# EI-CoreBioinformatics/portcullis

Measured on AMD Instinct MI355X. Metric: junc_reads_per_sec, higher is better.
Workload: dtype int32; 1 GPU; BASELINE configs[2]: synthetic 199999998 paired-end 150-bp reads, 25 contigs of GRCh38 lengths (3088286401 bp), 249999 junctions, orientation FR; reads_total=199999998, junctions_total=249999, contigs=25, reads_rank0=199999998, pairs_rank0=66692850

## Files before the change

### portcullis_amd/csrc/pjb_api.hip

```cpp
#include "pjb_host.hip.h"
#include "pjb_kernels.hip.h"
#include "pjb_chain.hip.h"

static int slot_init(pjb_ctx *c, int k);
static void aux_streams(pjb_ctx *c) {
    if (!c->stream3) (void)hipStreamCreateWithFlags(&c->stream3, hipStreamNonBlocking);
    if (!c->stream4) (void)hipStreamCreateWithFlags(&c->stream4, hipStreamNonBlocking);
}

extern "C" {

namespace {
std::mutex g_host_mu;
std::map<void *, size_t> g_host_registered;
}
void *pjb_host_alloc(size_t bytes) {
    if (bytes >= ((size_t)8 << 20)) {
        const size_t huge = (size_t)2 << 20, len = (bytes + huge - 1) & ~(huge - 1);
        void *p = mmap(nullptr, len, PROT_READ | PROT_WRITE, MAP_PRIVATE | MAP_ANONYMOUS, -1, 0);
        if (p != MAP_FAILED) {
            (void)madvise(p, len, MADV_HUGEPAGE);
            const size_t nt = std::min<size_t>(4, len >> 24);
            auto touch = [&](size_t t) {
                const size_t per = ((len / std::max<size_t>(nt, 1)) + huge - 1) & ~(huge - 1), a = std::min(len, per * t), b = std::min(len, a + per);
// ... 99 lines not shown
        (void)hipFuncSetAttribute((const void *)rs_scatter<0, u64>, hipFuncAttributeMaxDynamicSharedMemorySize, (int)rs_scatter_lds_bytes(RS_MAX_BITS));
        (void)hipFuncSetAttribute((const void *)rs_scatter<0, u32>, hipFuncAttributeMaxDynamicSharedMemorySize, (int)rs_scatter_lds_bytes(RS_MAX_BITS, 4));
    };
    std::thread attr_thread(attributes);
    struct JoinAttr {
        std::thread &t;
        ~JoinAttr() {
            if (t.joinable()) t.join();
        }
    } join_attr{attr_thread};
    c->cfg = *cfg;
    memset(&c->timing, 0, sizeof c->timing);
    e = hipStreamCreateWithFlags(&c->stream, hipStreamNonBlocking);
    if (e != hipSuccess) {
        delete c;
        return fail(nullptr, PJB_ERR_HIP, "hipStreamCreate: %s", hipGetErrorString(e));
    }
    if (!(cfg->flags & PJB_FLAG_NO_CHAINS)) aux_streams(c);
    (void)hipEventCreateWithFlags(&c->ev_front, hipEventDisableTiming);
    c->scan_tiles = &c->b_scan_tiles;
    cmark("main streams");
    if (!(cfg->flags & PJB_FLAG_NO_CHAINS))
        for (int k = 0; k < 4 && k < PJB_MAX_QUEUED; k++) (void)slot_init(c, k);
    cmark("chain slots");
    c->inflate_lanes = std::max(1, n_cu) * (160 * 1024 / ingest_lds_bytes()) * 64;
    c->ktime = (cfg->flags & PJB_FLAG_KERNEL_TIMING) != 0;
    c->extra = (cfg->flags & PJB_FLAG_EXTRA) != 0;
    if (const char *s = getenv("PJB_K1_SERIAL")) c->k1_serial = atoi(s) != 0;
    if (const char *s = getenv("PJB_K1S_BLOCKS")) c->k1s_blocks_forced = std::max(0, std::min(atoi(s), (int)K1S_BLOCKS));
    if (const char *s = getenv("PJB_RADIX_BITS")) {
        int v = atoi(s);
        if (v >= 4 && v <= RS_MAX_BITS) c->radix_max_bits = v;
    }
    cmark("options");
    attr_thread.join();
    cmark("kernel attributes");
    *out = c;
    return PJB_OK;
}


void pjb_destroy(pjb_ctx *c) {
    if (!c) return;
    (void)hipSetDevice(c->cfg.device);
    (void)hipDeviceSynchronize();
    (void)exhume(c);
#ifdef K1E_PROF
    {
        unsigned long long h[16] = {0};
        (void)hipDeviceSynchronize();
        if (hipMemcpyFromSymbol(h, HIP_SYMBOL(pjb::g_k1e_prof), sizeof h) == hipSuccess) {
            unsigned long long tot = 0;
            for (int i = 0; i < 12; i++) tot += h[i];
            static const char *nm[12] = {"block start", "prologue", "shapes (wait ops)", "windows issue", "next records issue", "stage wait", "next ops issue", "compare+emit", "lists", "cand flush", "span of bases", "bases issue"};
            for (int i = 0; i < 12; i++) fprintf(stderr, "[k1e_prof] %-20s %6.2f %%  %llu\n", nm[i], tot ? 100.0 * (double)h[i] / (double)tot : 0.0, h[i]);
        }
    }
#endif
    while (!c->open.empty()) close_contig(c, c->open.begin()->first);
    extra_clear(c);
    for (auto &kv : c->filter_keys)
        if (kv.second.first) (void)hipFree(kv.second.first);
    c->filter_keys.clear();
    for (auto &g : c->contigs) free_contig(g);
    for (auto &b : c->genome_pool) release(b);
    c->genome_pool.clear();
    for (auto &sl : c->slab_pool)
        if (sl.p) (void)hipFree(sl.p);
    if (c->rows_pinned) (void)hipHostFree(c->rows_pinned);
    if (c->rows_table) (void)hipFree(c->rows_table);
    bam_stage_clear(c);
    for (int k = 0; k < PJB_MAX_QUEUED; k++) {
        CtlSlot &S = c->sl[k];
        if (S.pub) (void)hipHostFree(S.pub);
        if (S.batches_pinned) (void)hipHostFree(S.batches_pinned);
        for (auto &ev : S.ev)
            if (ev) (void)hipEventDestroy(ev);
        if (S.ev_rows) (void)hipEventDestroy(S.ev_rows);
        if (S.ev_done) (void)hipEventDestroy(S.ev_done);
        Buf *sb[] = {&S.x_q, &S.x_spos, &S.x_send, &S.x_gapoff, &S.x_zlist, &S.x_scnt, &S.x_codes, &S.cstats, &S.err, &S.gencount, &S.batches, &S.rows, &S.tile_cnt, &S.tile_stats, &S.splidx, &S.splpoff, &S.splrec, &S.tile_soff, &S.chunk_tile, &S.scan_parts, &S.members, &S.okey, &S.g,
                     &S.rec, &S.jidbam, &S.jkey, &S.total, &S.bitmap, &S.wrank, &S.pagecnt, &S.pagerank, &S.ends, &S.firstid,
                     &S.key[0], &S.key[1], &S.idx[0], &S.idx[1], &S.hist, &S.hist_scan, &S.hist_part, &S.bintotal, &S.scan_tiles, &S.jid, &S.seg, &S.runfirst,
                     &S.runstart, &S.ent, &S.entsum, &S.frag, &S.fragj, &S.masks, &S.acc, &S.ancl, &S.ancr, &S.genlist, &S.runs};
        for (Buf *b : sb) release(*b);
        hipEvent_t evs[] = {S.ev_k1, S.ev_xk1, S.ev_fork, S.ev_join, S.ev_fork2, S.ev_join2};
        for (hipEvent_t e : evs)
            if (e) (void)hipEventDestroy(e);
        if (S.main) (void)hipStreamDestroy(S.main);
// ... 911 lines not shown
        if (b > a) c->ktime_only.push_back(s.substr(a, b - a));
        a = b + 1;
    }
    return PJB_OK;
}

int pjb_reset_kernel_timing(pjb_ctx *c) {
    if (!c) return PJB_ERR_ARG;
    std::fill(c->kcount.begin(), c->kcount.end(), 0);
    std::fill(c->kms.begin(), c->kms.end(), 0.0);
    return PJB_OK;
}

int pjb_set_option(pjb_ctx *c, const char *name, int64_t value) {
    if (!c || !name) return PJB_ERR_ARG;
    if (c->n_fl) return fail(c, PJB_ERR_STATE, "set_option: target %d is still queued", c->fl[0].tid);
    const std::string n = name;
    if (n == "overlap") c->side_stream = value != 0;
    else if (n == "dense_ids") c->dense_ids = value != 0;
    else if (n == "extra_dense") c->extra_dense_only = value != 0;
    else if (n == "sort_floor") c->sort_floor = (u32)std::max<int64_t>(1, std::min<int64_t>(value, 1 << 30));
    else if (n == "window_skip") c->window_skip = value != 0;
    else if (n == "run_sort") c->run_sort = value != 0;
    else if (n == "run_window") {
        if (value < 0 || value > (int64_t)RUN_W) return fail(c, PJB_ERR_ARG, "set_option: run_window takes 0 (the default, %u) to %u", RUN_W, RUN_W);
        c->run_window = (u32)value;
    } else if (n == "grow_batch") {
        if (value < 0 || value > 32768) return fail(c, PJB_ERR_ARG, "set_option: grow_batch takes 0 (the default: what the pool holds) to 32768 trees");
        c->model.grow_batch = (u32)value;
    } else if (n == "knn_chunk") {
        if (value < 0 || value > (1 << 22)) return fail(c, PJB_ERR_ARG, "set_option: knn_chunk takes 0 (the default: sized to fill the chip) to %d base rows", 1 << 22);
        c->model.knn_chunk = (u32)value;
    } else if (n == "list_cap") c->list_cap_forced = (u32)std::max<int64_t>(0, std::min<int64_t>(value, 1 << 30));
    else return fail(c, PJB_ERR_ARG, "set_option: unknown option '%s'", name);
    return PJB_OK;
}

int pjb_get_timing(const pjb_ctx *c, pjb_timing *out) {
    if (!c || !out) return PJB_ERR_ARG;
    if (c->cfg.abi_version >= 4) *out = c->timing;
    else memcpy(out, &c->timing, offsetof(pjb_timing, repeats));
    return PJB_OK;
}

}
```

### portcullis_amd/csrc/pjb_chain.hip.h

```cpp
#pragma once

constexpr unsigned K6_BLOCKS = 128;

static size_t rows_upper_bound(const pjb_ctx *c) {
    size_t n = c->rows_n;
    for (int k = 0; k < c->n_fl; k++)
        if (c->fl[k].queued) n += c->fl[k].lim.junc_limit;
    return n;
}

static void wait_flight(pjb_ctx *c, Flight &f) {
    if (f.queued) (void)hipEventSynchronize(c->sl[f.slot].ev_done);
}

static int rows_table_reserve(pjb_ctx *c, Flight &f, u32 JL) {
    size_t old = rows_upper_bound(c);
    if (old + JL <= c->rows_cap) return PJB_OK;
    for (int k = 0; k < c->n_fl; k++)
        if (c->fl[k].queued && &c->fl[k] != &f) wait_flight(c, c->fl[k]);
    int rc = rows_sync(c);
    if (rc) return rc;
    old = std::min(old, c->rows_cap);
    const size_t ncap = std::max<size_t>((old + JL) * 3 / 2, 1024);
    pjb_junction_row *nd = nullptr;
// ... 338 lines not shown
    }
    LAUNCH(c, "k1_scan_tiles", k1_scan_tiles, dim3(c->k1s_blocks_forced ? (u32)c->k1s_blocks_forced : k1s_blocks(n_tiles)), dim3(K1S_THREADS), (u32 *)S.tile_cnt.p, (const TileStats *)S.tile_stats.p,
           n_tiles, ch.d_cs, ch.PL, kf, ch.group ? INT32_MAX - 1 : ch.ref_len, (const u64 *)nullptr, (u32 *)S.tile_soff.p, (u32 *)S.chunk_tile.p,
           (ScanPart *)S.scan_parts.p, ++S.scan_epoch, c->window_skip ? 1u : 0u);
    EmitLists el;
    el.cand = f.lim.dense ? (u64 *)S.key[1].p : (u64 *)nullptr;
    el.bitmap = f.lim.dense ? (u64 *)S.bitmap.p : (u64 *)nullptr;
    el.page_cnt = f.lim.dense ? (u32 *)S.pagecnt.p : (u32 *)nullptr;
    el.cand_anc = (u64 *)S.ent.p;
    el.gen_list = (u64 *)S.genlist.p;
    el.gen_cnt = ch.d_gen_cnt;
    el.gen_cap = ch.gen_cap;
    el.pack_nn = ch.pack_nn;
    for (size_t b0 = 0; b0 < batches.size(); b0 += K1E_MAXB) {
        const size_t nb = std::min<size_t>(K1E_MAXB, batches.size() - b0);
        u64 reads = 0;
        for (size_t bi = b0; bi < b0 + nb; bi++) reads += (u64)batches[bi].n;
        const u32 nt = (u32)std::min<u64>((reads + K1_TILE - 1) / K1_TILE + nb, 0x7fffffffu);
        static const u32 tiles_per_block = getenv("PJB_K1E_TILES") ? (u32)std::max(1, atoi(getenv("PJB_K1E_TILES"))) : 8u;
        const u32 grid = std::max<u32>(1, std::min<u32>(nt, std::max<u32>(1024, nt / tiles_per_block)));
        LAUNCH(c, "k1_emit", k1_emit, dim3(grid), dim3(256), (const DevBatch *)S.batches.p + b0, (int)nb, n_tiles, (const u32 *)S.tile_cnt.p,
               (const u32 *)S.tile_soff.p, (const u32 *)S.chunk_tile.p, (const u32 *)S.splidx.p, (const u32 *)S.splpoff.p, (const uint4 *)S.splrec.p, ch.pr, el, kf,
               GT, ch.fast_codes ? 1 : 0, (int)c->cfg.orientation, ch.d_err, ch.d_cs);
    }
    if (c->k1_serial && !k1_late) {
        HIP_TRY(c, hipEventRecord(S.ev_k1, st));
        c->last_k1_ev = S.ev_k1;
    }
    if (ch.group)
        LAUNCH(c, "kg_member_stats", kg_member_stats, dim3((unsigned)ch.n_members), dim3(256), (const u32 *)S.tile_cnt.p, (const TileStats *)S.tile_stats.p,
               (const u32 *)ch.d_tile_lo, ch.n_members, ch.d_members, n_tiles, (const ContigStats *)ch.d_cs);
    LAUNCH(c, "k1_generic", k1_generic, dim3(std::min<u32>(std::max<u32>(1, (u32)(((u64)ch.gen_cap * GEN_SHARDS + K1E_T - 1) / K1E_T)), 1536u )), dim3(K1E_T),
           (const DevBatch *)S.batches.p, (int)batches.size(), (const u32 *)S.splidx.p, (const uint4 *)S.splrec.p, ch.pr, el, kf, GT, ch.fast_codes ? 1 : 0,
           (int)c->cfg.orientation, ch.d_err, ch.d_cs);
    if (c->k1_serial && k1_late) {
        HIP_TRY(c, hipEventRecord(S.ev_k1, st));
        c->last_k1_ev = S.ev_k1;
    }
    STAGE_EVENT(1);
    return PJB_OK;
}

static int chain_k4b(Chain &ch) {
    pjb_ctx *c = ch.c;
    CtlSlot &S = ch.S;
    const u32 gen_grid = std::min<u32>(2 * (u32)(((u64)ch.gen_cap * GEN_SHARDS + 255) / 256), 2560u);
    LAUNCH(c, "k4b_generic", k4b_generic, dim3(gen_grid), dim3(256), (const u64 *)S.genlist.p, (const u32 *)ch.d_gen_cnt, ch.gen_cap, (const u64 *)ch.pr.key,
           ch.pr.rec, (const u32 *)S.jidbam.p, ch.kf, (const DevBatch *)S.batches.p, (int)ch.f.batches.size(), (const int32_t *)S.ancl.p, (const int32_t *)S.ancr.p,
           ch.GT, ch.any_x ? 1 : 0, ch.any_x ? 0 : 1, ch.d_err, (const ContigStats *)ch.d_cs, ch.pack_nn, (const u32 *)S.splidx.p, (const uint4 *)S.splrec.p);
    return PJB_OK;
}

static int chain_k2d(Chain &ch) {
    pjb_ctx *c = ch.c;
    Flight &f = ch.f;
    CtlSlot &S = ch.S;
    if (!f.lim.dense) return PJB_OK;
    const KeyFmt kf = ch.kf;
    const u32 JL = ch.JL;
    const size_t n_words = ch.n_words;
    int rc;
    const u32 cand_blocks = std::min<u32>(ch.pair_blocks, 1024u);
    const u64 *okey = (const u64 *)ch.pr.key;
    u64 *cand = (u64 *)S.key[1].p;
    const u32 n_pages = (u32)((n_words + ((size_t)1 << KD_PAGE_SHIFT) - 1) >> KD_PAGE_SHIFT);
    if ((rc = run_scan(c, "kd_rank", ArrU32Fn{(const u32 *)S.pagecnt.p}, ExclusiveU32Sink{(u32 *)S.pagerank.p}, (u64)n_pages, (u64 *)S.total.p)))
        return rc;
// ... 241 lines not shown
```

### portcullis_amd/csrc/pjb_device.hip.h

```cpp
#pragma once

#include <hip/hip_runtime.h>
#include <stdint.h>

#include "../../include/portcullis_amd.h"

namespace pjb {

typedef unsigned long long u64;
typedef unsigned int u32;

struct DevBatch {
    const int32_t *pos;
    const uint16_t *flag;
    const uint8_t *mapq;
    const uint8_t *xs;
    const int32_t *l_qseq;
    const int32_t *mtid;
    const int32_t *mpos;
    const uint32_t *cig_off;
    const uint32_t *cigar;
    const uint32_t *seq_off;
    const uint8_t *seq4;
    const u64 *name_hash;
// ... 64 lines not shown
__device__ __forceinline__ void rec_store(PairRec *dst, const PairRec &r) {
    uint4 *q = reinterpret_cast<uint4 *>(dst);
    q[0] = make_uint4((u32)r.aux, (u32)(r.aux >> 32), (u32)r.lstart, (u32)r.rend);
    q[1] = make_uint4((u32)r.pos, (u32)r.aend, r.meta, r.updown);
}
__device__ __forceinline__ PairRec rec_load(const PairRec *src) {
    const uint4 *q = reinterpret_cast<const uint4 *>(src);
    const uint4 a = q[0], b = q[1];
    PairRec r;
    r.aux = (u64)a.x | ((u64)a.y << 32);
    r.lstart = (int32_t)a.z;
    r.rend = (int32_t)a.w;
    r.pos = (int32_t)b.x;
    r.aend = (int32_t)b.y;
    r.meta = b.z;
    r.updown = b.w;
    return r;
}

enum : u32 {
    META_CAT_MASK = 3u,
    META_MULTI = 1u << 2,
    META_XS_SHIFT = 3,
    META_UM = 1u << 5,
    META_BPP = 1u << 6,
    META_PPP = 1u << 7,
    META_REL = 1u << 8,
    META_SIMPLE = 1u << 9,
};
__device__ __forceinline__ u64 pack_res(u32 minMatch, u32 mmes, u32 mis) {
    return (u64)(minMatch & 0xfffffu) | ((u64)(mmes & 0xfffffu) << 20) | ((u64)mis << 40);
}
constexpr u32 RES_FIELD_MAX = 0xfffffu;

constexpr int GROUP_MAX = 32;
constexpr int32_t GROUP_GAP = 4096;
struct GroupTab {
    int32_t n;
    int32_t voff[GROUP_MAX];
    int32_t len[GROUP_MAX];
    int32_t tid[GROUP_MAX];
    const uint8_t *d[GROUP_MAX];
    const u32 *codes[GROUP_MAX];
    const u32 *codes2[GROUP_MAX];
    u32 exc_members;
};
struct Member {
    int32_t idx, voff, len, tid;
    const uint8_t *d;
    const u32 *codes;
};
__device__ __forceinline__ Member member_of(const GroupTab &T, int32_t vpos) {
    int m = 0;
    if (T.n > 1) {
#pragma unroll
        for (int s = GROUP_MAX / 2; s >= 1; s >>= 1)
            if (m + s < T.n && T.voff[m + s] <= vpos) m += s;
    }
    Member M;
    M.idx = m;
    M.voff = T.voff[m];
    M.len = T.len[m];
    M.tid = T.tid[m];
    M.d = T.d[m];
    M.codes = T.codes[m];
    return M;
// ... 427 lines not shown
```

### portcullis_amd/csrc/pjb_host.hip.h

```cpp
#pragma once
#include "pjb_device.hip.h"
#include "pjb_extra_types.hip.h"

#include <algorithm>
#include <sys/mman.h>
#include <thread>
#include <chrono>
#include <cstdarg>
#include <cstdio>
#include <cstdlib>
#include <cstring>
#include <map>
#include <memory>
#include <mutex>
#include <string>
#include <thread>
#include <vector>

using namespace pjb;


inline thread_local std::string g_create_error;
inline thread_local std::string g_thread_error;
inline thread_local const void *g_thread_error_ctx = nullptr;
// ... 224 lines not shown
    std::vector<Slab> slab_pool;
    uint8_t *stage[2] = {nullptr, nullptr};
    size_t stage_cap[2] = {0, 0};
    hipEvent_t stage_ev[2] = {nullptr, nullptr};
    bool stage_busy[2] = {false, false};
    unsigned stage_next = 0;
    pjb_junction_row *rows_pinned = nullptr;
    pjb_junction_row *rows_table = nullptr;
    bool rows_copy_pending = false;
    int last_slot = 0;
    int inflate_lanes = 512 * 64;
    bool side_stream = true;
    bool dense_ids = true;
    u32 junc_seen = 0;
    int lbits_seen = 18;
    size_t rows_n = 0, rows_cap = 0;
    size_t rows_pinned_cap = 0;
    std::vector<void *> graveyard;
    std::mutex grave_mu;
    size_t last_rows_n = 0;
    uint8_t *mirror = nullptr;
    size_t mirror_cap = 0;
    int64_t *mirror_hdr = nullptr;
    size_t mirror_rows = 0;
    int64_t mirror_acc[5] = {0, 0, 0, INT32_MAX, 0};
    pjb_timing timing;
    int radix_max_bits = 11;
    double junc_per_read = 0;
    u32 sort_floor = 1u << 16;
    bool window_skip = true;
    bool run_sort = true;
    u32 run_window = 0;
    u32 list_cap_forced = 0;
    bool k1_serial = true;
    hipEvent_t last_k1_ev = nullptr;
    int k1s_blocks_forced = 0;
    bool ktime = false;
    std::vector<std::string> knames;
    std::vector<int64_t> kcount;
    std::vector<double> kms;
    std::vector<std::string> ktime_only;
    Buf *scan_tiles = nullptr;
    Buf b_scan_tiles;
    Buf b_inf_comp, b_inf_out, b_inf_blocks, b_inf_status, b_inf_scratch, b_inf_bitmap;
    Buf b_dfl_in, b_dfl_sym, b_dfl_slots, b_dfl_size, b_dfl_off, b_dfl_packed;
    Buf b_bam_seg, b_bam_rec, b_bam_ctl;
    struct IndexState *index = nullptr;
    bool extra = false;
    std::vector<ExtraContig> xc;
    std::map<int32_t, std::pair<u64 *, u32>> filter_keys;
    Buf f_pos, f_cigoff, f_cigar, f_codes;
    ModelState model;
    Buf x_pos, x_endx, x_q, x_prefq, x_ce, x_bound, x_de, x_dropped, x_zlist, x_cnt, x_tabk, x_tabc, x_rs, x_re, x_rr, x_tileoff;
    Buf x_xrall, x_tab;
    size_t x_tab_slots = 0, x_tab_n = 0;
    XArena xarena;
    pjb_extra_row *xrows_pinned = nullptr;
    size_t xrows_pinned_cap = 0;
    bool extra_dense_only = false;
    Buf b_hasx, b_xtotal;
    Buf b_fasta_raw;
};


inline int fail(pjb_ctx *c, int code, const char *fmt, ...) {
    char tmp[1024];
// ... 316 lines not shown
```

### portcullis_amd/csrc/pjb_kernels.hip.h

```cpp
#pragma once

#include "pjb_device.hip.h"

namespace pjb {

__global__ __launch_bounds__(256) void k0_upper(uint8_t *g, int64_t n, int do_upper, int *has_x) {
    int64_t i = ((int64_t)blockIdx.x * 256 + threadIdx.x) * 16;
    bool x = false;
    for (int64_t j = i; j < n && j < i + 16; j++) {
        uint8_t c = g[j];
        x |= (c == 'X' || (do_upper && c == 'x'));
    }
    if (__ballot(x) && lane_id() == 0) atomicOr(has_x, 1);
    if (!do_upper) return;
    if (i + 16 <= n && ((uintptr_t)(g + i) & 15) == 0) {
        uint4 v = *reinterpret_cast<uint4 *>(g + i);
        u32 *w = reinterpret_cast<u32 *>(&v);
#pragma unroll
        for (int k = 0; k < 4; k++) {
            u32 x = w[k], r = 0;
#pragma unroll
            for (int b = 0; b < 4; b++) {
                u32 c = (x >> (8 * b)) & 0xff;
                if (c >= 'a' && c <= 'z') c -= 32;
// ... 878 lines not shown
}
constexpr int GEN_MAXB = 256;
struct BatchTab {
    u32 tbase[GEN_MAXB], seqw[GEN_MAXB], cigw[GEN_MAXB];
    __device__ __forceinline__ void fill(const DevBatch *batches, int n_batches) {
        if ((int)threadIdx.x < n_batches && threadIdx.x < (u32)GEN_MAXB) {
            const PJB_GLOBAL DevBatch *d = as_global(batches + threadIdx.x);
            tbase[threadIdx.x] = d->tile_base;
            seqw[threadIdx.x] = as_global(d->seq_off)[d->n];
            cigw[threadIdx.x] = as_global(d->cig_off)[d->n];
        }
    }
    __device__ __forceinline__ int find(const DevBatch *batches, int n_batches, u32 tile) const {
        int lo = 0, hi = n_batches - 1;
        if (n_batches <= GEN_MAXB) {
            while (lo < hi) {
                const int mid = (lo + hi + 1) >> 1;
                if (tbase[mid] <= tile) lo = mid;
                else hi = mid - 1;
            }
        } else {
            while (lo < hi) {
                const int mid = (lo + hi + 1) >> 1;
                if (gload(&batches[mid].tile_base) <= tile) lo = mid;
                else hi = mid - 1;
            }
        }
        return lo;
    }
    __device__ __forceinline__ u32 seq_words(const DevBatch &b, int bi) const { return bi < GEN_MAXB ? seqw[bi] : gload(b.seq_off + b.n); }
    __device__ __forceinline__ u32 cig_words(const DevBatch &b, int bi) const { return bi < GEN_MAXB ? cigw[bi] : gload(b.cig_off + b.n); }
};

struct NCursor {
    u32 i;
    int32_t acc;
    bool has;
    int32_t peek;
};
template <typename Ops>
__device__ __forceinline__ void ncursor_advance(NCursor &c, const Ops cig, u32 n) {
    c.has = false;
    while (c.i < n) {
        u32 op = cig[c.i++];
        u32 ty = op & 15u;
        if (op_consumes_ref(ty)) c.acc += (int32_t)(op >> 4);
        if (ty == OP_N) {
            c.has = true;
            c.peek = c.acc;
            return;
        }
    }
}

constexpr int SIMPLE_NW = 8;
struct CmpBlock {
    int32_t len, mism, first, last;
};
__device__ __forceinline__ u64 cmp_blocks_res(const CmpBlock &L, const CmpBlock &R) {
    const u32 upM = L.last < 0 ? (u32)L.len : (u32)(L.len - 1 - L.last);
    const u32 downM = R.first < 0 ? (u32)R.len : (u32)R.first;
    const u32 tu = (u32)(L.len - L.mism), td = (u32)(R.len - R.mism);
    return pack_res(upM < downM ? upM : downM, tu < td ? tu : td, (u32)(L.mism + R.mism));
}
struct EmitRead {
    u32 n;
// ... 58 lines not shown
            if (rStart - 1 >= ref_len) rStart = ref_len - 1;
            const int32_t iend = rStart - 1;
            while (U.has && U.peek < istart) {
                cntU++;
                ncursor_advance(U, cig, n);
            }
            while (D.has && D.peek <= iend + 1) {
                cntD++;
                ncursor_advance(D, cig, n);
            }
            const int64_t idx = (int64_t)R.off + k;
            const u64 key = make_key(kf, istart, iend);
            P.key[idx] = key;
            if (P.g) P.g[idx] = g;
            pend.lstart = lStart;
            pend.updown = cntU | ((nN - cntD) << 16);
            if (lStart > istart) set_error(err, g, PJB_ERR_MIN_ANCHOR);
            prev = idx;
            prev_key = key;
            blkL = blk;
            blk = Block{0, 0, -1, -1};
            prevIstart = istart;
            prevQ = qAcc;
            prevIend = iend;
            prevRStartU = rStartU;
            sumAfter = 0;
            lStart = rStart;
            lEndExc = rStart;
            k++;
        } else {
            if (closed && ty != OP_S) {
                const bool cq = op_consumes_query(ty), cr = op_consumes_ref(ty);
                if (cq && cr)
                    cmp_words<SIMPLE_NW, true>(R.closed_seqw, qAcc, R.q_limit, R.gcodes, lEndExc - R.voff, (R.glen + 7) / 8 + 1, ln, blk.len, blk.mism, blk.first, blk.last);
                else {
                    blk.mism += ln;
                    if (blk.first < 0) blk.first = blk.len;
                    blk.last = blk.len + ln - 1;
                }
                blk.len += ln;
            }
            if (op_consumes_ref(ty)) {
                lEndExc += ln;
                sumAfter += ln;
            }
        }
        if (op_consumes_query(ty)) qAcc += ln;
    }
    if (prev >= 0) {
        int32_t rEndExc = prevRStartU + sumAfter;
        if (rEndExc - 1 >= ref_len) rEndExc = ref_len;
        pend.rend = rEndExc - 1;
        if (closed) pend.aux = closed_stats();
        rec_store(P.rec + prev, pend);
        on_pair(prev_key, pend.lstart, pend.rend);
        if (rEndExc - 1 < prevIend) set_error(err, g, PJB_ERR_MIN_ANCHOR);
    }
}

__device__ __forceinline__ u32 read_meta(u32 flag, u32 xs, u32 mapq, int32_t pos, int32_t mtid, int32_t mpos, int32_t tid, int orientation) {
    const bool pp_check = orientation == PJB_OR_FR || orientation == PJB_OR_RF || orientation == PJB_OR_FF;
    const bool first = flag & 0x40, rev = flag & 0x10;
    u32 meta = (first ? 0u : 2u) + (rev ? 1u : 0u);
    meta |= (xs & 3u) << META_XS_SHIFT;
    const bool um = mapq >= 30;
    if (um) meta |= META_UM;
    if (flag & 0x2) meta |= META_BPP;
    bool ppp = false;
    if (pp_check) {
        const bool paired = flag & 0x1, mate_mapped = !(flag & 0x8);
        if (paired && mate_mapped && tid == mtid) {
            const bool mrev = flag & 0x20;
            const bool diff = rev != mrev;
            const bool gap = !rev ? pos < mpos : pos > mpos;
            ppp = orientation == PJB_OR_FR ? (diff && gap) : orientation == PJB_OR_RF ? (diff && !gap) : (!diff && gap);
        }
    }
    if (ppp) meta |= META_PPP;
    if (um && (!pp_check || ppp)) meta |= META_REL;
    return meta;
}

constexpr int K1E_LOOK = 16;
#ifndef K1E_WAVES
#define K1E_WAVES 4
#endif
constexpr int K1E_T = 256, K1E_SHIFT = 8;
constexpr int KC_SLOTS = K1E_T;
constexpr u64 KD_EMPTY = ~0ull;
// ... 348 lines not shown
            const u32 n = O.n;
            const u32 (&op)[OPS_LDS] = O.op;
            g = b.base + R.r;
            off = R.toff + R.poff;
            meta = read_meta(O.flag, O.xs, O.mapq, pos, O.mtid, O.mpos, tid, orientation);
            const bool seq_ok = (R.sr.w & 0x8000u) != 0;
            if (gcodes != nullptr && n >= 3 && n <= 7) {
                const bool clipF = (op[0] & 15u) == OP_S;
                const u32 i0 = clipF ? 1u : 0u;
                const u32 oa = clipF ? op[1] : op[0], on_ = clipF ? op[2] : op[1], ob = clipF ? op[3] : op[2];
                const u32 o3 = clipF ? op[4] : op[3], o4 = clipF ? op[5] : op[4], o5 = clipF ? op[6] : op[5];
                two = n >= i0 + 5u && (o3 & 15u) == OP_N;
                const u32 body = i0 + (two ? 5u : 3u);
                const u32 oL = two ? o5 : o3;
                const bool clipL = n == body + 1u && (oL & 15u) == OP_S;
                if (n == body || clipL) {
                    dS = clipF ? op[0] >> 4 : 0u;
                    const u32 dE = clipL ? oL >> 4 : 0u;
                    a = oa >> 4;
                    nl = on_ >> 4;
                    b2 = ob >> 4;
                    nl2 = two ? o3 >> 4 : 0u;
                    b3 = two ? o4 >> 4 : 0u;
                    simple = (oa & 15u) == OP_M && (on_ & 15u) == OP_N && (ob & 15u) == OP_M && a > 0 && b2 > 0 && a <= RES_FIELD_MAX && b2 <= RES_FIELD_MAX &&
                             dS <= RES_FIELD_MAX && lq > 1 && (u64)lq == (u64)dS + a + b2 + b3 + dE && seq_ok;
                    if (two)
                        simple = simple && (o4 & 15u) == OP_M && b3 > 0 && b3 <= RES_FIELD_MAX && nl > 0 && nl2 > 0 && pos >= 0 &&
                                 (int64_t)pos + a + nl + b2 + nl2 + b3 <= (int64_t)ref_len;
                }
            }
            two = two && simple;
            chk2 = two && window_reach(b2, nl, nl2, max_span);
            generic = !simple;
        }
        const u32 shard = (chunk >> (8 - K1E_SHIFT)) % GEN_SHARDS;
        const u32 base2 = ctx.list_reserve(2, chk2, 2u, shard), base3 = ctx.list_reserve(3, generic, 0u, shard);
        K1E_MARK(2);
        bool use2 = simple && gcodes2 != nullptr && !((O.excw >> (R.r & 31u)) & 1u) && pos >= 0 && (int64_t)pos + a + nl + b2 + nl2 + b3 <= (int64_t)ref_len &&
                    a <= (u32)C2_MAX_BLOCK && b2 <= (u32)C2_MAX_BLOCK && b3 <= (u32)C2_MAX_BLOCK;
        const int64_t n2w = codes2_words(ref_len);
        const bool any_exc = (G.exc_members >> mem) & 1u;
        Words2 x0 = {0, 0}, x1 = {0, 0}, x2 = {0, 0};
        if (use2 && any_exc) {
            const PJB_GLOBAL u32 *gexc = gcodes2 + n2w + K0_CODES2_PAD;
            const u32 g1 = (u32)pos + a + nl;
            x0 = gload_as<Words2>(gexc + ((u32)pos >> 11));
            x1 = gload_as<Words2>(gexc + (g1 >> 11));
            if (two) x2 = gload_as<Words2>(gexc + ((g1 + b2 + nl2) >> 11));
        }
        const bool more = v + 1 < v_hi, more2 = v + 2 < v_hi;
        EmitTrip T2 = T1;
        EmitRec R2 = R1;
        EmitOps On = O;
        if (more2) {
            T2 = locate(v + 2);
            R2 = fetch_rec(T2);
        }
        K1E_MARK(4);
        if (more) On = fetch_ops(T1, R1);
        K1E_MARK(6);
        const u32 *seqw = (const u32 *)b.seq4 + so;
        const int32_t q_limit = (int32_t)min(seq_words - 1u - so, 0x7fffffffu);
        if (simple) {
            const int32_t vpos = pos + voff;
            const int32_t aend_all = vpos + (int32_t)(a + nl + b2 + nl2 + b3) - 1;
            const u32 npairs = two ? 2u : 1u;
// ... 108 lines not shown
            for (u32 pr = 0; pr < 2; pr++) {
                if (pr >= npairs) break;
                PairRec Q;
                Q.lstart = lst_[pr];
                Q.rend = rend_[pr];
                Q.pos = vpos;
                Q.aend = aend_all;
                Q.meta = meta | META_SIMPLE | (two ? META_MULTI : 0u);
                Q.updown = ud_[pr];
                Q.aux = cmp_blocks_res(res[pr], res[pr + 1]);
                const u64 key = make_key(kf, ist_[pr], iend_[pr]);
                P.key[off + pr] = key;
                if (want_g) P.g[off + pr] = g;
                rec_store(P.rec + off + pr, Q);
                if (want_cand) cand_insert(key, Q.lstart, Q.rend);
            }
        }
        const u64 p1_entry = (u64)(E.pack_nn ? R.slot | (2u << 28) : R.slot) | ((u64)off << 32);
        K1E_MARK(7);
        ctx.list_write(2, chk2, base2, p1_entry, shard);
        ctx.list_write(3, generic, base3, (u64)R.slot | ((u64)off << 32), shard);
        K1E_MARK(8);
        if (!more) ctx.cand_flush(true);
        K1E_MARK(9);
        T = T1;
        R = R1;
        O = On;
        T1 = T2;
        R1 = R2;
    }
}

__global__ __launch_bounds__(K1E_T) void k1_generic(const DevBatch *batches, int n_batches, const u32 *spl_idx, const uint4 *spl_rec, Pairs P, EmitLists E, KeyFmt kf,
                                                    GroupTab G, int use_codes, int orientation, u64 *err, ContigStats *cs) {
    __shared__ EmitShared sh;
    __shared__ u32 s_ops[OPS_LDS][K1E_T];
    __shared__ u32 s_first[GEN_SHARDS + 1];
    __shared__ u32 s_wsum[4];
    __shared__ BatchTab s_bt;
    if (cs->P == 0) return;
    const u32 max_span = cs->max_span;
    const bool want_cand = E.cand != nullptr;
    EmitCtx ctx{sh, E, kf, cs, want_cand};
    ctx.init();
    static_assert(GEN_SHARDS == K1E_T, "a sub-list per thread");
    {
        const u32 c = E.gen_cnt[threadIdx.x * GEN_CNT_STRIDE + 4];
        s_bt.fill(batches, n_batches);
        u32 total;
        const u32 ex = block_escan<K1E_T / 64>(c < E.gen_cap ? c : E.gen_cap, s_wsum, &total);
        s_first[threadIdx.x] = ex;
        if (threadIdx.x == K1E_T - 1) s_first[GEN_SHARDS] = total;
        __syncthreads();
    }
    const u32 n_items = s_first[GEN_SHARDS];
    for (u32 item0 = blockIdx.x * K1E_T; item0 < n_items; item0 += gridDim.x * K1E_T) {
        const u32 item = item0 + threadIdx.x;
        u32 gen_pairs = 0, gen_kind = 0;
        u64 gen_entry = 0;
        if (item < n_items) {
            u32 sub = 0;
#pragma unroll
            for (u32 step = GEN_SHARDS / 2; step > 0; step >>= 1)
                if (sub + step < GEN_SHARDS && s_first[sub + step] <= item) sub += step;
            const u64 e3 = E.gen_list[((size_t)2 * GEN_SHARDS + sub) * E.gen_cap + (item - s_first[sub])];
            const u32 slot = (u32)e3;
            const int bi = s_bt.find(batches, n_batches, slot / (u32)K1_TILE);
            const DevBatch &b = batches[bi];
            const u32 r = spl_idx[slot];
            const uint4 sr = spl_rec[slot];
            const int m = b.member;
            const int32_t voff = G.voff[m], ref_len = G.len[m], vlen = voff + ref_len;
            const u32 *gcodes = use_codes ? G.codes[m] : (const u32 *)nullptr;
            EmitRead R;
            R.n = sr.w & 0x7fffu;
            if (R.n == 0x7fffu) R.n = gload(b.cig_off + r + 1) - sr.x;
            R.lq = (int32_t)(sr.w >> 16);
            if (R.lq == 0xffff) R.lq = gload(b.l_qseq + r);
            const int32_t pos = (int32_t)sr.y;
            R.pos = pos + voff;
            R.g = b.base + r;
            R.meta = read_meta(gload(b.flag + r), (u32)gload(b.xs + r), gload(b.mapq + r), pos, gload(b.mtid + r), gload(b.mpos + r), G.tid[m], orientation);
            R.seq_ok = (sr.w & 0x8000u) != 0;
            R.off = (u32)(e3 >> 32);
            OpsViewT<K1E_T, OPS_LDS> cig;
            cig.g = b.cigar + sr.x;
            cig.lds = &s_ops[0][threadIdx.x];
            {
                u32 w[OPS_LDS];
                fetch_ops8(as_global(b.cigar), sr.x, s_bt.cig_words(b, bi), w);
#pragma unroll
                for (int q = 0; q < OPS_LDS; q++) s_ops[q][threadIdx.x] = (u32)q < R.n ? w[q] : 0u;
            }
            u32 nN = 0, shape = 0;
            int32_t aligned = 0;
            int64_t qsum = 0, bsum = 0;
            u32 bref = 0, nl_prev = 0;
            bool reach = max_span == 0xffffffffu;
            for (u32 q = 0; q < R.n; q++) {
                const u32 o = cig[q], ty = o & 15u, ln = o >> 4;
                if (ty == OP_N) {
                    if (nN > 0) reach = reach || window_reach(bref, nl_prev, ln, max_span);
                    nl_prev = ln;
                    bref = 0;
                } else if (op_consumes_ref(ty))
                    bref = __builtin_elementwise_add_sat(bref, ln);
                nN += (ty == OP_N);
                if (op_consumes_ref(ty)) aligned += (int32_t)ln;
                if (op_consumes_query(ty)) qsum += ln;
                const bool len_ok = ln > 0 && ln <= RES_FIELD_MAX;
                if (ty == OP_M || ty == OP_EQ || ty == OP_X) shape = (shape == 0 || shape == 5 || shape == 2 || shape == 1 || shape == 6) && len_ok ? 1u : 4u;
                else if (ty == OP_I || ty == OP_D) shape = shape == 1 && len_ok ? 6u : 4u;
                else if (ty == OP_N) shape = shape == 1 && ln > 0 ? 2u : 4u;
                else if (ty == OP_S) shape = shape == 0 && len_ok ? 5u : shape == 1 && q + 1 == R.n ? 3u : 4u;
                else shape = 4;
                bsum = ty == OP_N ? 0 : ty == OP_S ? bsum : bsum + ln;
                if (bsum > (int64_t)RES_FIELD_MAX) shape = 4;
            }
            if (nN > 1) R.meta |= META_MULTI;
            R.nN = nN;
            R.aend = R.pos + aligned - 1;
            const bool closed = gcodes != nullptr && (shape == 1 || shape == 3) && nN > 0 && R.seq_ok && R.lq > 1 && qsum == (int64_t)R.lq &&
                                R.pos >= voff && R.aend < vlen;
            R.closed_seqw = closed ? reinterpret_cast<const u32 *>(b.seq4) + sr.z : nullptr;
            R.q_limit = (int32_t)min(s_bt.seq_words(b, bi) - 1u - sr.z, 0x7fffffffu);
            R.gcodes = gcodes;
            R.glen = ref_len;
            R.voff = voff;
            emit_read_pairs(cig, R, P, kf, vlen, err, [&](u64 key, int32_t lstart, int32_t rend) { ctx.cand_insert(key, lstart, rend); });
            gen_pairs = nN;
            gen_kind = !closed ? 1u : reach ? 2u : 0u;
            gen_entry = (u64)(closed && E.pack_nn ? slot | ((nN < 15u ? nN : 15u) << 28) : slot) | ((u64)R.off << 32);
        }
        const u32 shard = (item0 >> K1E_SHIFT) % GEN_SHARDS;
        ctx.list_append(1, gen_kind == 1, gen_pairs, gen_entry, shard);
        ctx.list_append(2, gen_kind == 2, gen_pairs, gen_entry, shard);
        ctx.cand_flush(item0 + gridDim.x * K1E_T >= n_items);
    }
}

__global__ __launch_bounds__(256) void kg_member_stats(const u32 *tile_off, const TileStats *ts, const u32 *tile_lo, int n_members, MemberStats *out, u32 n_tiles,
                                                       const ContigStats *cs) {
    __shared__ u64 sm[4][4];
    __shared__ int32_t smi[4][2];
    const int m = blockIdx.x;
    if (m >= n_members) return;
    u64 spl = 0, uns = 0, sum = 0, pairs = 0;
    int32_t mn = INT32_MAX, mx = 0;
    for (u32 t = tile_lo[m] + threadIdx.x; t < tile_lo[m + 1]; t += 256) {
        const TileStats x = ts[t];
        spl += x.spliced;
        uns += x.unspliced;
        sum += x.sum_len;
        mn = min(mn, x.min_len);
        mx = max(mx, x.max_len);
    }
    spl = wave_sum(spl);
    uns = wave_sum(uns);
    sum = wave_sum(sum);
    {
        const u32 t0 = tile_lo[m], t1 = tile_lo[m + 1], total = (u32)cs->n_pairs;
        pairs = threadIdx.x == 0 ? (u64)((t1 < n_tiles ? tile_off[t1] : total) - (t0 < n_tiles ? tile_off[t0] : total)) : 0ull;
    }
    mn = wave_min(mn);
    mx = wave_max(mx);
    const int w = threadIdx.x >> 6;
    if (lane_id() == 0) {
        sm[w][0] = spl;
        sm[w][1] = uns;
        sm[w][2] = sum;
// ... 1555 lines not shown
```

Measured before the change: 30.03 billion reads/s.

## Split generic closed-read comparisons into wave-uniform segment rounds in k1_generic

For closed generic reads with at most K1G_SEGS match segments, the kernel first walks the CIGAR to emit pair keys and stores segment lengths and gap kinds in LDS. A separate loop then compares read against reference chunk by chunk, advancing all lanes of the wavefront together instead of each lane running its own cigar walk with embedded comparisons. The aim is to cut divergence in the compare phase. In addition, read metadata is now precomputed in the earlier kernel and stored in P.rec, so k1_generic no longer reloads flag, mapq and mate fields. The change adds 16 LDS words per thread, which may lower occupancy, and brings in an optional profiling build with a rounds knob.

```diff
diff --git a/portcullis_amd/csrc/pjb_api.hip b/portcullis_amd/csrc/pjb_api.hip
--- a/portcullis_amd/csrc/pjb_api.hip
+++ b/portcullis_amd/csrc/pjb_api.hip
@@ -155,6 +155,9 @@
         int v = atoi(s);
         if (v >= 4 && v <= RS_MAX_BITS) c->radix_max_bits = v;
     }
+#ifdef K1G_PROF
+    if (const char *s = getenv("PJB_K1G_ROUNDS")) c->generic_rounds = (u32)std::max(0, std::min(atoi(s), (int)K1G_SEGS));
+#endif
     cmark("options");
     attr_thread.join();
     cmark("kernel attributes");
@@ -177,6 +180,19 @@
             for (int i = 0; i < 12; i++) tot += h[i];
             static const char *nm[12] = {"block start", "prologue", "shapes (wait ops)", "windows issue", "next records issue", "stage wait", "next ops issue", "compare+emit", "lists", "cand flush", "span of bases", "bases issue"};
             for (int i = 0; i < 12; i++) fprintf(stderr, "[k1e_prof] %-20s %6.2f %%  %llu\n", nm[i], tot ? 100.0 * (double)h[i] / (double)tot : 0.0, h[i]);
+        }
+    }
+#endif
+#ifdef K1G_PROF
+    {
+        unsigned long long h[8] = {0};
+        (void)hipDeviceSynchronize();
+        if (hipMemcpyFromSymbol(h, HIP_SYMBOL(pjb::g_k1g_prof), sizeof h) == hipSuccess) {
+            const unsigned long long v[6] = {h[0], h[1], h[2], h[3] > h[6] ? h[3] - h[6] : 0, h[4] + h[6], h[5]};
+            unsigned long long tot = 0;
+            for (int i = 0; i < 6; i++) tot += v[i];
+            static const char *nm[6] = {"list entry, spl_idx/rec", "predicates", "ops to LDS, shape", "walk w/o compares", "compares", "appends, cand flush"};
+            for (int i = 0; i < 6; i++) fprintf(stderr, "[k1g_prof] %-24s %6.2f %%  %llu\n", nm[i], tot ? 100.0 * (double)v[i] / (double)tot : 0.0, v[i]);
         }
     }
 #endif
@@ -1154,6 +1170,7 @@
         if (value < 0 || value > (1 << 22)) return fail(c, PJB_ERR_ARG, "set_option: knn_chunk takes 0 (the default: sized to fill the chip) to %d base rows", 1 << 22);
         c->model.knn_chunk = (u32)value;
     } else if (n == "list_cap") c->list_cap_forced = (u32)std::max<int64_t>(0, std::min<int64_t>(value, 1 << 30));
+    else if (n == "generic_rounds") c->generic_rounds = (u32)std::max<int64_t>(0, std::min<int64_t>(value, K1G_SEGS));
     else return fail(c, PJB_ERR_ARG, "set_option: unknown option '%s'", name);
     return PJB_OK;
 }
diff --git a/portcullis_amd/csrc/pjb_chain.hip.h b/portcullis_amd/csrc/pjb_chain.hip.h
--- a/portcullis_amd/csrc/pjb_chain.hip.h
+++ b/portcullis_amd/csrc/pjb_chain.hip.h
@@ -394,7 +394,7 @@
                (const u32 *)ch.d_tile_lo, ch.n_members, ch.d_members, n_tiles, (const ContigStats *)ch.d_cs);
     LAUNCH(c, "k1_generic", k1_generic, dim3(std::min<u32>(std::max<u32>(1, (u32)(((u64)ch.gen_cap * GEN_SHARDS + K1E_T - 1) / K1E_T)), 1536u )), dim3(K1E_T),
            (const DevBatch *)S.batches.p, (int)batches.size(), (const u32 *)S.splidx.p, (const uint4 *)S.splrec.p, ch.pr, el, kf, GT, ch.fast_codes ? 1 : 0,
-           (int)c->cfg.orientation, ch.d_err, ch.d_cs);
+           ch.d_err, ch.d_cs, c->generic_rounds);
     if (c->k1_serial && k1_late) {
         HIP_TRY(c, hipEventRecord(S.ev_k1, st));
         c->last_k1_ev = S.ev_k1;
diff --git a/portcullis_amd/csrc/pjb_device.hip.h b/portcullis_amd/csrc/pjb_device.hip.h
--- a/portcullis_amd/csrc/pjb_device.hip.h
+++ b/portcullis_amd/csrc/pjb_device.hip.h
@@ -120,6 +120,7 @@
     return (u64)(minMatch & 0xfffffu) | ((u64)(mmes & 0xfffffu) << 20) | ((u64)mis << 40);
 }
 constexpr u32 RES_FIELD_MAX = 0xfffffu;
+constexpr int K1G_SEGS = 8;
 
 constexpr int GROUP_MAX = 32;
 constexpr int32_t GROUP_GAP = 4096;
diff --git a/portcullis_amd/csrc/pjb_host.hip.h b/portcullis_amd/csrc/pjb_host.hip.h
--- a/portcullis_amd/csrc/pjb_host.hip.h
+++ b/portcullis_amd/csrc/pjb_host.hip.h
@@ -280,6 +280,7 @@
     bool run_sort = true;
     u32 run_window = 0;
     u32 list_cap_forced = 0;
+    u32 generic_rounds = K1G_SEGS;
     bool k1_serial = true;
     hipEvent_t last_k1_ev = nullptr;
     int k1s_blocks_forced = 0;
diff --git a/portcullis_amd/csrc/pjb_kernels.hip.h b/portcullis_amd/csrc/pjb_kernels.hip.h
--- a/portcullis_amd/csrc/pjb_kernels.hip.h
+++ b/portcullis_amd/csrc/pjb_kernels.hip.h
@@ -934,6 +934,27 @@
     __device__ __forceinline__ u32 cig_words(const DevBatch &b, int bi) const { return bi < GEN_MAXB ? cigw[bi] : gload(b.cig_off + b.n); }
 };
 
+#ifdef K1G_PROF
+__device__ unsigned long long g_k1g_prof[8];
+#define K1G_T0() unsigned long long gprof_t = __builtin_amdgcn_s_memtime()
+#define K1G_MARK(i)                                                                  \
+    do {                                                                             \
+        const unsigned long long now_ = __builtin_amdgcn_s_memtime();                \
+        if (lane_id() == 0) atomicAdd(&g_k1g_prof[i], now_ - gprof_t);               \
+        gprof_t = now_;                                                              \
+    } while (0)
+#define K1G_CMP(stmt)                                                                                                     \
+    do {                                                                                                                  \
+        const unsigned long long c0_ = __builtin_amdgcn_s_memtime();                                                      \
+        stmt;                                                                                                             \
+        const unsigned long long c1_ = __builtin_amdgcn_s_memtime();                                                      \
+        if (lane_id() == __ffsll((long long)__ballot(1)) - 1) atomicAdd(&g_k1g_prof[6], c1_ - c0_);                       \
+    } while (0)
+#else
+#define K1G_T0() do {} while (0)
+#define K1G_MARK(i) do {} while (0)
+#define K1G_CMP(stmt) stmt
+#endif
 struct NCursor {
     u32 i;
     int32_t acc;
@@ -1058,7 +1079,7 @@
             if (closed && ty != OP_S) {
                 const bool cq = op_consumes_query(ty), cr = op_consumes_ref(ty);
                 if (cq && cr)
-                    cmp_words<SIMPLE_NW, true>(R.closed_seqw, qAcc, R.q_limit, R.gcodes, lEndExc - R.voff, (R.glen + 7) / 8 + 1, ln, blk.len, blk.mism, blk.first, blk.last);
+                    K1G_CMP((cmp_words<SIMPLE_NW, true>(R.closed_seqw, qAcc, R.q_limit, R.gcodes, lEndExc - R.voff, (R.glen + 7) / 8 + 1, ln, blk.len, blk.mism, blk.first, blk.last)));
                 else {
                     blk.mism += ln;
                     if (blk.first < 0) blk.first = blk.len;
@@ -1081,6 +1102,115 @@
         rec_store(P.rec + prev, pend);
         on_pair(prev_key, pend.lstart, pend.rend);
         if (rEndExc - 1 < prevIend) set_error(err, g, PJB_ERR_MIN_ANCHOR);
+    }
+}
+
+constexpr u32 SEG_GAP_NONE = 0, SEG_GAP_I = 1, SEG_GAP_D = 2, SEG_GAP_N = 3, SEG_GAP_SHIFT = 20;
+static_assert(RES_FIELD_MAX < (1u << SEG_GAP_SHIFT), "a segment's length and its gap's kind share a word");
+template <int STRIDE, typename Ops, typename PairFn>
+__device__ __forceinline__ int32_t closed_pairs_walk(const Ops cig, const EmitRead R, const Pairs P, const KeyFmt kf, const int32_t ref_len, u64 *err,
+                                                     u32 *seg, PairFn &&on_pair) {
+    const u32 n = R.n, g = R.g, nN = R.nN;
+    int32_t lStart = R.pos, lEndExc = R.pos, prevIend = 0, q0 = 0;
+    int64_t prev = -1;
+    u64 prev_key = 0;
+    PairRec pend;
+    pend.lstart = pend.rend = 0;
+    pend.pos = R.pos;
+    pend.aend = R.aend;
+    pend.meta = R.meta | META_SIMPLE;
+    pend.updown = 0;
+    u32 k = 0, s = 0, gap = SEG_GAP_NONE, gap_len = 0;
+    auto finish = [&]() {
+        pend.rend = lEndExc - 1;
+        reinterpret_cast<uint2 *>(P.rec + prev)[1] = make_uint2((u32)pend.lstart, (u32)pend.rend);
+        reinterpret_cast<uint4 *>(P.rec + prev)[1] = make_uint4((u32)pend.pos, (u32)pend.aend, pend.meta, pend.updown);
+        on_pair(prev_key, pend.lstart, pend.rend);
+        if (pend.rend < prevIend) set_error(err, g, PJB_ERR_MIN_ANCHOR);
+    };
+    for (u32 i = 0; i < n; i++) {
+        const u32 op = cig[i];
+        const u32 ty = op & 15u;
+        const int32_t ln = (int32_t)(op >> 4);
+        if (ty == OP_N) {
+            if (prev >= 0) finish();
+            const int32_t istart = lEndExc, iend = lEndExc + ln - 1;
+            const int64_t idx = (int64_t)R.off + k;
+            const u64 key = make_key(kf, istart, iend);
+            P.key[idx] = key;
+            if (P.g) P.g[idx] = g;
+            pend.lstart = lStart;
+            pend.updown = k | ((nN - k - 1u) << 16);
+            if (lStart > istart) set_error(err, g, PJB_ERR_MIN_ANCHOR);
+            prev = idx;
+            prev_key = key;
+            prevIend = iend;
+            lStart = lEndExc = iend + 1;
+            gap = SEG_GAP_N;
+            gap_len = (u32)ln;
+            k++;
+        } else if (ty == OP_S) {
+            if (i == 0) q0 = ln;
+        } else if (ty == OP_I || ty == OP_D) {
+            gap = ty == OP_I ? SEG_GAP_I : SEG_GAP_D;
+            gap_len = (u32)ln;
+            if (ty == OP_D) lEndExc += ln;
+        } else {
+            seg[(2 * s) * STRIDE] = (u32)ln | (gap << SEG_GAP_SHIFT);
+            seg[(2 * s + 1) * STRIDE] = gap_len;
+            s++;
+            gap = SEG_GAP_NONE;
+            gap_len = 0;
+            lEndExc += ln;
+        }
+    }
+    if (prev >= 0) finish();
+    return q0;
+}
+template <int STRIDE>
+__device__ __forceinline__ void closed_rounds(const u32 *seg, u32 nsegs, const u32 *seqw, int32_t q_limit, const u32 *gcodes, int32_t g_words, int32_t q0, int32_t g0,
+                                              PairRec *rec) {
+    u32 s = 0, kblk = 0;
+    int32_t qi = q0, gi = g0, t = 0, ob = 0;
+    int32_t l = nsegs ? (int32_t)(seg[0] & RES_FIELD_MAX) : 0;
+    u32 mism = 0, fbit = 0xffffffffu, lbit1 = 0;
+    CmpBlock L = {0, 0, -1, -1};
+    while (__ballot(s < nsegs)) {
+        if (s < nsegs) {
+            CmpChunkT<SIMPLE_NW> C;
+            chunk_load<SIMPLE_NW, true>(C, seqw, qi, q_limit, gcodes, gi, g_words, l, t);
+            u32 fb = 0xffffffffu, lb = 0;
+            chunk_cmp_bits<SIMPLE_NW>(C, qi, gi, l, t, mism, fb, lb);
+            fbit = min(fbit, __builtin_elementwise_add_sat(fb, 4u * (u32)ob));
+            lbit1 = lb ? lb + 4u * (u32)ob : lbit1;
+            t += 8 * (SIMPLE_NW - 1);
+            if (t >= l) {
+                qi += l, gi += l, ob += l;
+                s++;
+                bool block_ends = s == nsegs;
+                if (s < nsegs) {
+                    const u32 w = seg[(2 * s) * STRIDE], gl = seg[(2 * s + 1) * STRIDE], kind = w >> SEG_GAP_SHIFT;
+                    if (kind == SEG_GAP_I || kind == SEG_GAP_D) {
+                        mism += gl;
+                        fbit = min(fbit, 4u * (u32)ob + 3u);
+                        lbit1 = 4u * ((u32)ob + gl);
+                        ob += (int32_t)gl;
+                    }
+                    if (kind == SEG_GAP_I) qi += (int32_t)gl;
+                    if (kind == SEG_GAP_D || kind == SEG_GAP_N) gi += (int32_t)gl;
+                    block_ends = kind == SEG_GAP_N;
+                    l = (int32_t)(w & RES_FIELD_MAX);
+                    t = 0;
+                }
+                if (block_ends) {
+                    const CmpBlock B = {ob, (int32_t)mism, (int32_t)fbit >> 2, ((int32_t)lbit1 - 1) >> 2};
+                    if (kblk > 0) *reinterpret_cast<u64 *>(rec + (kblk - 1)) = cmp_blocks_res(L, B);
+                    L = B;
+                    kblk++;
+                    ob = 0, mism = 0, fbit = 0xffffffffu, lbit1 = 0;
+                }
+            }
+        }
     }
 }
 
@@ -1495,6 +1625,7 @@
             two = two && simple;
             chk2 = two && window_reach(b2, nl, nl2, max_span);
             generic = !simple;
+            if (generic) P.rec[off].meta = meta;
         }
         const u32 shard = (chunk >> (8 - K1E_SHIFT)) % GEN_SHARDS;
         const u32 base2 = ctx.list_reserve(2, chk2, 2u, shard), base3 = ctx.list_reserve(3, generic, 0u, shard);
@@ -1669,9 +1800,10 @@
 }
 
 __global__ __launch_bounds__(K1E_T) void k1_generic(const DevBatch *batches, int n_batches, const u32 *spl_idx, const uint4 *spl_rec, Pairs P, EmitLists E, KeyFmt kf,
-                                                    GroupTab G, int use_codes, int orientation, u64 *err, ContigStats *cs) {
+                                                    GroupTab G, int use_codes, u64 *err, ContigStats *cs, u32 rounds) {
     __shared__ EmitShared sh;
     __shared__ u32 s_ops[OPS_LDS][K1E_T];
+    __shared__ u32 s_seg[2 * K1G_SEGS][K1E_T];
     __shared__ u32 s_first[GEN_SHARDS + 1];
     __shared__ u32 s_wsum[4];
     __shared__ BatchTab s_bt;
@@ -1695,6 +1827,11 @@
         const u32 item = item0 + threadIdx.x;
         u32 gen_pairs = 0, gen_kind = 0;
         u64 gen_entry = 0;
+        u32 nsegs = 0;
+        const u32 *r_seqw = nullptr, *r_gcodes = nullptr;
+        int32_t r_qlimit = 0, r_gwords = 0, r_q0 = 0, r_g0 = 0;
+        PairRec *r_rec = nullptr;
+        K1G_T0();
         if (item < n_items) {
             u32 sub = 0;
 #pragma unroll
@@ -1717,9 +1854,11 @@
             const int32_t pos = (int32_t)sr.y;
             R.pos = pos + voff;
             R.g = b.base + r;
-            R.meta = read_meta(gload(b.flag + r), (u32)gload(b.xs + r), gload(b.mapq + r), pos, gload(b.mtid + r), gload(b.mpos + r), G.tid[m], orientation);
+            K1G_MARK(0);
+            R.meta = gload(&P.rec[(u32)(e3 >> 32)].meta);
             R.seq_ok = (sr.w & 0x8000u) != 0;
             R.off = (u32)(e3 >> 32);
+            K1G_MARK(1);
             OpsViewT<K1E_T, OPS_LDS> cig;
             cig.g = b.cigar + sr.x;
             cig.lds = &s_ops[0][threadIdx.x];
@@ -1729,7 +1868,7 @@
 #pragma unroll
                 for (int q = 0; q < OPS_LDS; q++) s_ops[q][threadIdx.x] = (u32)q < R.n ? w[q] : 0u;
             }
-            u32 nN = 0, shape = 0;
+            u32 nN = 0, shape = 0, nseg = 0;
             int32_t aligned = 0;
             int64_t qsum = 0, bsum = 0;
             u32 bref = 0, nl_prev = 0;
@@ -1746,6 +1885,7 @@
                 if (op_consumes_ref(ty)) aligned += (int32_t)ln;
                 if (op_consumes_query(ty)) qsum += ln;
                 const bool len_ok = ln > 0 && ln <= RES_FIELD_MAX;
+                nseg += (ty == OP_M || ty == OP_EQ || ty == OP_X);
                 if (ty == OP_M || ty == OP_EQ || ty == OP_X) shape = (shape == 0 || shape == 5 || shape == 2 || shape == 1 || shape == 6) && len_ok ? 1u : 4u;
                 else if (ty == OP_I || ty == OP_D) shape = shape == 1 && len_ok ? 6u : 4u;
                 else if (ty == OP_N) shape = shape == 1 && ln > 0 ? 2u : 4u;
@@ -1764,15 +1904,31 @@
             R.gcodes = gcodes;
             R.glen = ref_len;
             R.voff = voff;
-            emit_read_pairs(cig, R, P, kf, vlen, err, [&](u64 key, int32_t lstart, int32_t rend) { ctx.cand_insert(key, lstart, rend); });
+            K1G_MARK(2);
+            auto on_pair = [&](u64 key, int32_t lstart, int32_t rend) { ctx.cand_insert(key, lstart, rend); };
+            if (closed && nseg <= min(rounds, (u32)K1G_SEGS)) {
+                r_q0 = closed_pairs_walk<K1E_T>(cig, R, P, kf, vlen, err, &s_seg[0][threadIdx.x], on_pair);
+                nsegs = nseg;
+                r_seqw = R.closed_seqw;
+                r_gcodes = gcodes;
+                r_qlimit = R.q_limit;
+                r_gwords = (ref_len + 7) / 8 + 1;
+                r_g0 = pos;
+                r_rec = P.rec + R.off;
+            } else
+                emit_read_pairs(cig, R, P, kf, vlen, err, on_pair);
+            K1G_MARK(3);
             gen_pairs = nN;
             gen_kind = !closed ? 1u : reach ? 2u : 0u;
             gen_entry = (u64)(closed && E.pack_nn ? slot | ((nN < 15u ? nN : 15u) << 28) : slot) | ((u64)R.off << 32);
         }
+        closed_rounds<K1E_T>(&s_seg[0][threadIdx.x], nsegs, r_seqw, r_qlimit, r_gcodes, r_gwords, r_q0, r_g0, r_rec);
+        K1G_MARK(4);
         const u32 shard = (item0 >> K1E_SHIFT) % GEN_SHARDS;
         ctx.list_append(1, gen_kind == 1, gen_pairs, gen_entry, shard);
         ctx.list_append(2, gen_kind == 2, gen_pairs, gen_entry, shard);
         ctx.cand_flush(item0 + gridDim.x * K1E_T >= n_items);
+        K1G_MARK(5);
     }
 }
 
```

Result: no change. 30.22 billion reads/s (median of 2 runs) (+0.6%).
